# daviyan5/ninpol

Measured on AMD Instinct MI355X. Metric: Mnodes/s interpolated (GLS, 10M-cell hex mesh) + achieved HBM GB/s vs peak, higher is better.
Workload: dtype f64

## Files before the change

ninpol_amd/csrc/abi_apply.hip:

```cpp
#include <hipcub/hipcub.hpp>

#include "abi_internal.hpp"
#include "gls_adjoint.hpp"

using namespace nin;

int nin::ensure_transpose_index(DeviceGrid &d, hipStream_t stream) {
    if (d.tr_cell_ptr) return NIN_OK;
    const int32_t E = d.v.n_elems, nnz = (int32_t)d.nnz_e;
    int32_t *&ptr = d.tr_cell_ptr, *&pos = d.tr_cell_pos, *&node = d.tr_cell_node;
    DevTmp<int32_t> cells_sorted;
    DevTmp<void> tmp;
    size_t tmp_bytes = 0;
    int end_bit = 1;
    while (end_bit < 31 && (int64_t{1} << end_bit) < (int64_t)E) ++end_bit;
    int rc = dev_alloc(d, &ptr, (size_t)E + 1);
    if (!rc) rc = dev_alloc(d, &pos, (size_t)nnz);
    if (!rc) rc = dev_alloc(d, &node, (size_t)nnz);
    auto step = [&](hipError_t e) { if (e != hipSuccess && rc == NIN_OK) rc = fail(NIN_EHIP, "transpose index: %s", hipGetErrorString(e)); return rc == NIN_OK; };
    if (!rc && nnz > 0) {
        if (step(hipMalloc((void **)&cells_sorted, (size_t)nnz * sizeof(int32_t))) &&
            step(launch_iota(node, nnz, stream) ? hipErrorLaunchFailure : hipSuccess) &&
            step(hipcub::DeviceRadixSort::SortPairs(nullptr, tmp_bytes, d.v.esup, cells_sorted.p, node, pos, nnz, 0, end_bit, stream)) &&
            step(hipMalloc(&tmp, tmp_bytes)) &&
// ... 18 lines not shown
                     double *dev_neumann_ws, void *stream_) {
    if (!g || !dev_u_cells || !dev_node_values || !dev_neumann_ws) return fail(NIN_EINVAL, "NULL argument");
    if (n_fields < 1) return fail(NIN_EINVAL, "n_fields must be >= 1");
    DeviceGrid &d = g->d;
    if (int rc = on_device(g, kHintWeights)) return rc;
    HIP_TRY(hipSetDevice(d.device));
    hipStream_t stream = static_cast<hipStream_t>(stream_);
    if (int rc = ensure_apply_weights(d)) return rc;
    const DeviceGrid::GlsList &cube = d.plan[gk::hex8];
    if (method == NIN_METHOD_GLS && cube.count > 0 && d.noncube_nodes_ready && getenv("NIN_APPLY_NO_FUSION") == nullptr) {
        int rc = weights_ready(d, method);
        if (rc) return rc;
        HIP_TRY(hipMemsetAsync(d.gls_queue, 0, kGlsQueueInts * sizeof(int32_t), stream));
        rc = gls_side_begin(d, -1, 1, d.apply_weights, dev_neumann_ws, stream);
        if (!rc) rc = launch_gls_hex8mf_apply(d.v, cube.nodes, reinterpret_cast<const int32_t *>(cube.desc), cube.count, 1, dev_u_cells, n_fields,
                                              dev_node_values, dev_neumann_ws, d.gls_queue + gls_plan_row(gk::hex8).counter, stream);
        if (!rc) rc = gls_main(d, -1, false, gls_only(), 1, d.apply_weights, dev_neumann_ws, stream);
        if (!rc) rc = launch_apply_list(d.v, d.apply_weights, dev_u_cells, n_fields, dev_node_values, d.noncube_nodes, d.noncube_count, stream);
        if (rc) return fail(rc, "launch failed: %s", hipGetErrorString(hipGetLastError()));
        return NIN_OK;
    }
    int rc = nin_weights_device(g, method, nullptr, 0, 1, d.apply_weights, dev_neumann_ws, stream_);
    if (rc) return rc;
    rc = n_fields == 1 ? launch_apply(d.v, d.apply_weights, dev_u_cells, dev_node_values, (int32_t)g->h.mx_elems_per_point, d.nnz_e, stream)
                       : launch_apply_fields(d.v, d.apply_weights, dev_u_cells, n_fields, dev_node_values, (int32_t)g->h.mx_elems_per_point, d.nnz_e, stream);
    if (rc) return fail(rc, "launch failed");
    return NIN_OK;
}

int nin_apply_fields_host(nin_grid *g, int method, const double *u_cells, int32_t n_fields, double *node_values,
                          double *neumann_ws) {
// ... 336 lines not shown
```

ninpol_amd/csrc/abi_plan.hip:

```cpp
#include <hipcub/hipcub.hpp>
#include <cmath>

#include "abi_internal.hpp"
#include "hex8_desc.hpp"
#include "mfw_desc.hpp"
#include "mfg_desc.hpp"
#include "mfx_desc.hpp"
#include "quad4_desc.hpp"

using namespace nin;

namespace {

#ifndef NIN_LOCALITY_RUN
#define NIN_LOCALITY_RUN 16
#endif
constexpr int kLocalityRun = NIN_LOCALITY_RUN;
__device__ __forceinline__ uint32_t spread10(uint32_t v) {
    v = (v | (v << 16)) & 0x030000FFu;
    v = (v | (v << 8)) & 0x0300F00Fu;
    v = (v | (v << 4)) & 0x030C30C3u;
    v = (v | (v << 2)) & 0x09249249u;
    return v;
}
// ... 76 lines not shown
        default: return 0;
    }
}

int launch_plan_kernel(const DeviceGrid &d, GlsKernel k, const int32_t *nodes, const uint32_t *desc, int32_t count, int add_neumann,
                       double *out, double *nws, hipStream_t stream) {
    const GlsPlanRow r = gls_plan_row(k);
    const DeviceGrid::GlsList &l = d.plan[k];
    int32_t *queue = r.counter >= 0 ? d.gls_queue + r.counter : nullptr;
    const int32_t *idesc = reinterpret_cast<const int32_t *>(desc);
    switch (r.family) {
        case GlsFamily::block: return launch_gls_block(d.v, nodes, count, l.waves, l.col_slots, l.lds_bytes, add_neumann, out, nws, queue, stream);
        case GlsFamily::scratch:
            return launch_gls_class(d.v, nodes, count, 0, l.rows_per_lane, add_neumann, out, nws, d.gls_scratch, d.gls_scratch_stride,
                                    d.gls_scratch_slots, stream);
        case GlsFamily::hex8: return launch_gls_hex8mf(d.v, nodes, idesc, count, add_neumann, out, nws, queue, stream);
        case GlsFamily::mfw: return launch_gls_mfw(d.v, nodes, desc, count, r.sub, add_neumann, out, nws, queue, stream);
        case GlsFamily::small: return launch_gls_small(d.v, nodes, count, r.sub, add_neumann, out, nws, stream);
        case GlsFamily::quad4: return launch_gls_quad4(d.v, nodes, idesc, count, add_neumann, out, nws, stream);
        case GlsFamily::mfx: return launch_gls_mfx(d.v, nodes, desc, count, r.sub, add_neumann, out, nws, queue, stream);
        case GlsFamily::mfg: return launch_gls_mfg(d.v, nodes, desc, count, add_neumann, out, nws, queue, d.mfg_tiles, d.mfg_slots, stream);
    }
    return NIN_EINVAL;
}

}

int nin::build_gls_plan(nin_grid *g) {
    DeviceGrid &d = g->d;
    const int64_t P = g->h.n_points;
    int rc;
// ... 59 lines not shown
        const int32_t *lp = nullptr;
        if ((rc = dev_upload(d, &lp, lists[k]))) return rc;
        l.nodes = const_cast<int32_t *>(lp);
        if (k == gk::hex8 && locality && (rc = locality_order(d, l.nodes, l.count, d.chunk_node))) return rc;
        if (const int words = gls_plan_row(k).desc_words) {
            if ((rc = dev_alloc(d, &l.desc, (size_t)l.count * words))) return rc;
            if (launch_plan_desc(d, GlsKernel(k), l.nodes, l.count, l.desc, nullptr)) return fail(NIN_EHIP, "descriptor kernel of plan kernel %d", k);
        }
    }
    if (d.plan[gk::mfg_tiles].count) {
        d.mfg_slots = std::min<int32_t>(d.plan[gk::mfg_tiles].count, kMfgResidentWaves);
        if ((rc = dev_alloc(d, &d.mfg_tiles, (size_t)d.mfg_slots * kMfgSlotDoubles))) return rc;
    }
    d.gls_too_large = rows_max[gk::scratch] > 1024;
    if ((rc = dev_alloc(d, &d.gls_queue, (size_t)kGlsQueueInts))) return rc;
    if (d.plan[gk::scratch].count) {
        d.gls_scratch_slots = std::min<int32_t>(d.plan[gk::scratch].count, 512);
        d.gls_scratch_stride = need_max[gk::scratch] / 8;
        if ((rc = dev_alloc(d, &d.gls_scratch, (size_t)d.gls_scratch_slots * d.gls_scratch_stride))) return rc;
    }
    const char *mn = getenv("NIN_E2E_MIN_NODES");
    d.chunkable = P >= (mn ? atoll(mn) : 64 * 1024) && P >= 64 * K && getenv("NIN_E2E_NO_PIPELINE") == nullptr;
    for (int c = 0; c < kGlsClasses; ++c)
        if (d.plan[c].count == P) { d.plan[c].nodes = nullptr; d.chunkable = false; }
    return NIN_OK;
}

static constexpr GlsKernel kSideOrder[] = {gk::mfg_tiles, gk::scratch};
static constexpr GlsKernel kMainOrder[] = {gk::hex8,     gk::mfw_large, gk::mfw_small, gk::mfw_general, gk::small4,       gk::small8,
                                           gk::small12,  gk::quad4,     gk::mfx_6x10,  gk::mfx_7x11,    gk::mfx_8x13,     gk::mfx_9x15,
                                           gk::mfx_10x16, gk::mfx_boundary, gk::mfx_4x7, gk::mfx_7x12,  gk::mfg_tiles,    gk::block1,
                                           gk::block2,   gk::block4,    gk::block8,    gk::scratch};
static constexpr bool main_order_is_complete() {
    unsigned seen = 0;
    for (GlsKernel k : kMainOrder) seen |= 1u << k;
    return sizeof kMainOrder / sizeof kMainOrder[0] == kGlsPlanKernels && seen == (1u << kGlsPlanKernels) - 1;
}
static_assert(main_order_is_complete(), "kMainOrder must name every kernel of the plan once");
static bool on_side_stream(GlsKernel k) { return std::find(std::begin(kSideOrder), std::end(kSideOrder), k) != std::end(kSideOrder); }

struct PlanRange { const int32_t *nodes; const uint32_t *desc; int32_t count; };
static PlanRange plan_range(const DeviceGrid &d, GlsKernel k, int piece) {
    const auto &l = d.plan[k];
    const int32_t b = piece < 0 ? 0 : l.chunk_off[piece], n = (piece < 0 ? l.count : l.chunk_off[piece + 1]) - b;
    return {l.nodes ? l.nodes + b : nullptr, l.desc ? l.desc + (size_t)gls_plan_row(k).desc_words * b : nullptr, n};
// ... 67 lines not shown
                       double *dev_csr_data, double *dev_neumann_ws, void *stream_) {
    if (!g || !dev_csr_data || !dev_neumann_ws) return fail(NIN_EINVAL, "NULL argument");
    DeviceGrid &d = g->d;
    int rc = on_device(g, kHintWeights);
    if (!rc) rc = weights_ready(d, method);
    if (rc) return rc;
    hipStream_t stream = static_cast<hipStream_t>(stream_);
    HIP_TRY(hipSetDevice(d.device));
    const int64_t P = g->h.n_points;
    const bool all = targets == nullptr;
    if (!all && n_targets < 0) return fail(NIN_EINVAL, "negative n_targets");
    if (all) {
        if (method == NIN_METHOD_IDW) rc = launch_idw(d.v, nullptr, (int32_t)P, (int32_t)g->h.mx_elems_per_point, d.nnz_e, dev_csr_data, dev_neumann_ws, stream);
        else if (method == NIN_METHOD_LS) rc = launch_ls(d.v, nullptr, (int32_t)P, (int32_t)g->h.mx_elems_per_point, d.nnz_e, dev_csr_data, dev_neumann_ws, stream);
        else {
            HIP_TRY(hipMemsetAsync(d.gls_queue, 0, kGlsQueueInts * sizeof(int32_t), stream));
            const int only = gls_only();
            if (only < 0) rc = gls_side_begin(d, -1, add_neumann, dev_csr_data, dev_neumann_ws, stream);
            if (!rc) rc = gls_main(d, -1, true, only, add_neumann, dev_csr_data, dev_neumann_ws, stream);
        }
        if (rc) return fail(rc, "kernel launch failed: %s", hipGetErrorString(hipGetLastError()));
        return NIN_OK;
    }
    for (int64_t i = 0; i < n_targets; ++i)
        if (targets[i] < 0 || targets[i] >= P) return fail(NIN_EINVAL, "target %lld out of range", (long long)targets[i]);
    HIP_TRY(hipMemsetAsync(dev_csr_data, 0, (size_t)d.nnz_e * 8, stream));
    HIP_TRY(hipMemsetAsync(dev_neumann_ws, 0, (size_t)P * 8, stream));
    if (n_targets == 0) return NIN_OK;
    const bool gls = method == NIN_METHOD_GLS;
    std::vector<int32_t> lists[kGlsPlanKernels];
    for (int64_t i = 0; i < n_targets; ++i) lists[gls ? gls_class_kernel(g->node_class[targets[i]]) : 0].push_back((int32_t)targets[i]);
// ... 158 lines not shown
```

ninpol_amd/csrc/device_grid.hpp:

```cpp
#pragma once
#include <cstdint>
#include <string>
#include <vector>

#include "gls_plan.hpp"

namespace nin {

struct GridView {
    int32_t n_points, n_elems, n_faces, dim;
    const int32_t *esup_ptr;
    const int32_t *esup;
    const int32_t *fsup_ptr;
    const int32_t *fsup;
    const double *coords;
    const double *centroids;
    const double *centroids4;
    const int32_t *face_cells;
    const double *face_center;
    const float *face_normal;
    const double *perm;
    const double *diff_mag;
    const uint8_t *flags;
};
// ... 6 lines not shown
    return ((doubles * 8 + 15) / 16) * 16;
}
NIN_HD inline int gls_node_class(int64_t ne, int64_t nf, int64_t nbf, bool force_global, int64_t *bytes, int64_t *rows,
                                 int64_t *cols) {
    const int64_t m = ne + 3 * (nf - nbf) + nbf, n = 3 * ne + 1;
    int c = kGlsClasses - 1;
    int64_t b = ((((ne + 1) >> 1) + n + m * n) * 8 + 15) / 16 * 16;
    for (int k = 0; k < kGlsClasses - 1 && !force_global && n <= 256; ++k) {
        const int64_t need = gls_block_lds_bytes(ne, m, n, gls_class_waves(k));
        if (need <= gls_class_budget(k)) { c = k; b = need; break; }
    }
    *bytes = b; *rows = m; *cols = n;
    return c;
}

struct DeviceGrid {
    int device = -1;
    GridView v{};
    int64_t nnz_e = 0, nnz_f = 0;
    bool fields_set = false, have_perm = false;
    bool prebuilt = false;
    std::vector<void *> allocs;

    static constexpr int kE2eChunks = 4;
    int32_t chunk_node[kE2eChunks + 1] = {0, 0, 0, 0, 0};
    bool chunkable = false;
    struct GlsList {
        int32_t count = 0;
        int32_t *nodes = nullptr;
        uint32_t *desc = nullptr;
        int32_t chunk_off[kE2eChunks + 1] = {};
        int32_t lds_bytes = 0;
        int32_t waves = 1;
        int32_t col_slots = 1;
        int32_t rows_per_lane = 1;
    } plan[kGlsPlanKernels];
    double *mfg_tiles = nullptr;
    int32_t mfg_slots = 0;
    const int32_t *noncube_nodes = nullptr;
    int32_t noncube_count = 0;
    bool noncube_nodes_ready = false;
    double *gls_scratch = nullptr;
    int64_t gls_scratch_stride = 0;
    int32_t gls_scratch_slots = 0;
    int32_t *gls_queue = nullptr;
    double *e2e_weights = nullptr, *e2e_nws = nullptr, *e2e_data = nullptr;
    int32_t *e2e_cnt = nullptr, *e2e_ptr = nullptr, *e2e_indices = nullptr;
    void *e2e_tmp = nullptr;
    size_t e2e_tmp_bytes = 0;
    double *apply_weights = nullptr;
    int32_t *tr_cell_ptr = nullptr, *tr_cell_pos = nullptr, *tr_cell_node = nullptr;
    struct AdjBin {
        int32_t count = 0;
        int32_t *nodes = nullptr;
        int64_t bytes = 0;
    } adj_bin[4];
    bool adj_ready = false;
    double *adj_contrib = nullptr, *adj_scratch = nullptr;
    int64_t adj_scratch_stride = 0;
    int32_t adj_scratch_slots = 0;
// ... 36 lines not shown
```

ninpol_amd/csrc/gls_plan.hpp:

```cpp
#pragma once
#include <cstdint>

#ifdef __HIPCC__
#define NIN_HD __host__ __device__
#else
#define NIN_HD
#endif

namespace nin {

constexpr int kGlsClasses = 5;

constexpr int kGlsPlanKernels = 22;
namespace gk {
enum GlsKernel : int {
    block1, block2, block4, block8, scratch,
    hex8,
    mfw_large, mfw_small, mfw_general,
    small4, small8, small12,
    quad4,
    mfx_6x10, mfx_7x11, mfx_8x13, mfx_9x15, mfx_10x16,
    mfx_boundary,
    mfg_tiles,
    mfx_4x7,
// ... 7 lines not shown
    scratch,
    hex8,
    mfw,
    small,
    quad4,
    mfx,
    mfg,
};

constexpr int kGlsQueueLine = 16;
constexpr int kGlsQueueHex8 = 0, kGlsQueueHex8Lines = 8;
constexpr int kGlsQueueBlock = 1;
constexpr int kGlsQueueMfw = 5;
constexpr int kGlsQueueMfx = 8, kGlsQueueMfxLists = 8;
constexpr int kGlsQueueMfg = 8 * kGlsQueueLine;
constexpr int kGlsQueueInts = 9 * kGlsQueueLine;
static_assert(kGlsQueueBlock > kGlsQueueHex8 && kGlsQueueBlock + (kGlsClasses - 1) <= kGlsQueueMfw, "block counters overlap");
static_assert(kGlsQueueMfw + 3 <= kGlsQueueMfx, "mfw counters overlap the mfx counters");
static_assert(kGlsQueueMfx + kGlsQueueMfxLists <= kGlsQueueLine, "the block / mfw / mfx counters must stay between hex8's ints 0 and 16");
static_assert(kGlsQueueMfg % kGlsQueueLine == 0 && kGlsQueueMfg / kGlsQueueLine >= kGlsQueueHex8 / kGlsQueueLine + kGlsQueueHex8Lines,
              "the mfg counter must lie on none of hex8's eight lines");
static_assert(kGlsQueueMfg < kGlsQueueInts, "the mfg counter lies outside the block");

struct GlsPlanRow {
    GlsFamily family;
    int8_t sub;
    uint8_t class_byte;
    int16_t desc_words;
    int16_t fdq_word;
    int16_t counter;
};
// ... 87 lines not shown
```

ninpol_amd/csrc/kernels_gls_hex8mf.hip:

```cpp
#include <hip/hip_runtime.h>

#include <cstdio>
#include <cstdlib>

#include "device_grid.hpp"
#include "gls_device_math.hpp"
#include "hex8_desc.hpp"
#include "launch.hpp"

namespace nin {

namespace {

using namespace glsmath;

__device__ __forceinline__ double quad_sum(double v) {
    v += dpp_mov<0xB1>(v);
    v += dpp_mov<0x4E>(v);
    return v;
}
template <int L>
__device__ __forceinline__ double quad_bcast(double v) { return dpp_mov<L * 0x55>(v); }

constexpr int NPW = 16;
// ... 86 lines not shown
        const bool own = R0 >= 0 && r >= R0 && r < R0 + 3;
        const double v = own ? fma(w0, P[r][0], b[own ? r - R0 : 0]) : w0 * P[r][0];
        fill[r - 3] = fma(w2, P[r][2], fma(w1, P[r][1], v));
    }
}

__device__ __forceinline__ void w2_dma16(const void *gptr, uint32_t *row) {
    __builtin_amdgcn_global_load_lds((const __attribute__((address_space(1))) void *)gptr, (__attribute__((address_space(3))) void *)row, 16, 0, 0);
}
__device__ __forceinline__ void w2_dma_wait() {
    __builtin_amdgcn_sched_barrier(0);
    asm volatile("s_waitcnt vmcnt(0)" ::: "memory");
    __builtin_amdgcn_sched_barrier(0);
}
constexpr int W2_REC_ROW = 256;
__device__ __forceinline__ void w2_stage_rec(const int32_t *rec, int32_t wg, int32_t count, int nd, int l, uint32_t *rows_r) {
    const int32_t idx = wg * NPW + nd;
    const uint32_t sel = (uint32_t)((idx >= 0 && idx < count) ? idx : count - 1);
    const int32_t *r = rec + kHex8LaneWords * (4 * (size_t)sel + l);
    w2_dma16(r, rows_r);
    w2_dma16(r + 4, rows_r + W2_REC_ROW);
}
struct W2Geo {
    double Ke[9], dme, ce[3];
    double Ko[9], dmo, co[3];
    double fc[3][3];
    float fn[3][3];
    double xv[3];
    uint32_t flags;
};
__device__ __forceinline__ void w2_stage_d(const GridView &g, const uint32_t *rows_r, int lane, W2Geo &q) {
    const uint4 ra = *reinterpret_cast<const uint4 *>(rows_r + 4 * lane);
    const uint4 rb = *reinterpret_cast<const uint4 *>(rows_r + W2_REC_ROW + 4 * lane);
#pragma unroll
    for (int t = 0; t < 3; ++t) q.xv[t] = g.coords[3 * (size_t)ra.x + t];
    q.flags = g.flags[ra.x];
    const uint32_t ce = ra.z, co = ra.w;
#pragma unroll
    for (int k = 0; k < 9; ++k) { q.Ke[k] = g.perm[9 * (size_t)ce + k]; q.Ko[k] = g.perm[9 * (size_t)co + k]; }
    q.dme = g.diff_mag[ce];
    q.dmo = g.diff_mag[co];
#pragma unroll
    for (int t = 0; t < 3; ++t) { q.ce[t] = g.centroids[3 * (size_t)ce + t]; q.co[t] = g.centroids[3 * (size_t)co + t]; }
#pragma unroll
    for (int i = 0; i < 3; ++i) {
        const uint32_t f = i == 0 ? rb.x : i == 1 ? rb.y : rb.z;
#pragma unroll
        for (int t = 0; t < 3; ++t) { q.fn[i][t] = g.face_normal[3 * (size_t)f + t]; q.fc[i][t] = g.face_center[3 * (size_t)f + t]; }
    }
}
template <int I>
__device__ __forceinline__ double w2_across(double v) { return dpp_mov<I == 0 ? 0x40 : I == 1 ? 0xA5 : 0xFE>(v); }

#ifndef W2_D_STEP
#define W2_D_STEP 6
#endif
static_assert(W2_D_STEP >= 0 && W2_D_STEP <= 12, "the geometry is requested in phase 2");

#ifdef NIN_W2_TRACE
__device__ unsigned long long nin_w2_trace[4096 * 4];
#endif
template <bool APPLY>
__global__ __launch_bounds__(256, 2) void nin_gls_hex8w2_kernel(GridView g, const int32_t *__restrict__ nodes,
                                                                const int32_t *__restrict__ desc, int32_t count,
                                                                int add_neumann, double *__restrict__ out,
                                                                double *__restrict__ nws, int32_t *__restrict__ queue,
                                                                const double *__restrict__ u_cells, int32_t n_fields,
                                                                double *__restrict__ values) {
    __shared__ __attribute__((aligned(16))) double lds_all[4][W2_WAVE_DOUBLES];
    static_assert(W2_WAVE_DOUBLES % 2 == 0, "a wave's slots begin on a 16-byte boundary (the records' rows)");
    __shared__ double tau_tab[TAU_TAB_DOUBLES];
    static_assert(2 * (sizeof(double) * (4 * W2_WAVE_DOUBLES + TAU_TAB_DOUBLES)) <= 160 * 1024, "two workgroups per CU");
    tau_table_to_lds(tau_tab);
    __syncthreads();
    const lds_cdouble_ptr tau_lds = (lds_cdouble_ptr)tau_tab;
    const int lane = threadIdx.x & 63, wave = threadIdx.x >> 6;
    const int l = lane & 3, nd = lane >> 2;
    double *const L = lds_all[wave] + lane;
    double *const wbuf = lds_all[wave] + W2_SLOTS * 64;
    uint32_t *const rows_r = reinterpret_cast<uint32_t *>(lds_all[wave] + 13 * 64);

    const int32_t n_groups = (count + NPW - 1) / NPW;
    int32_t wg_lo, wg_end;
    int32_t *q;
    if ((gridDim.x & 7) == 0) {
        const int32_t xcd = blockIdx.x & 7, per = (n_groups + 7) / 8;
        wg_lo = xcd * per;
        wg_end = (xcd + 1) * per < n_groups ? (xcd + 1) * per : n_groups;
        q = queue + kGlsQueueLine * xcd;
    } else {
        wg_lo = 0;
        wg_end = n_groups;
        q = queue;
    }
    int32_t ticket = 0;
    if (lane == 0) ticket = atomicAdd(q, 1);
    int32_t wg = wg_lo + __builtin_amdgcn_readfirstlane(ticket);
    if (lane == 0) ticket = atomicAdd(q, 1);
    int32_t wg_next = wg_lo + __builtin_amdgcn_readfirstlane(ticket);
    W2Geo geo;
    w2_stage_rec(desc, wg, count, nd, l, rows_r);
    w2_dma_wait();
    w2_stage_d(g, rows_r, lane, geo);
#ifdef NIN_MF_STAMPS
#ifndef NIN_MF_STAMP_PASS
#define NIN_MF_STAMP_PASS 8
#endif
    unsigned long long stamps[8];
    int n_stamp = 0, pass_no = 0;
#define NIN_MF_STAMP() do { if (n_stamp < 8) { __builtin_amdgcn_sched_barrier(0); stamps[n_stamp++] = __builtin_amdgcn_s_memtime(); __builtin_amdgcn_s_waitcnt(0xC07F); __builtin_amdgcn_sched_barrier(0); } } while (0)
#else
#define NIN_MF_STAMP() do { } while (0)
#endif
#ifdef NIN_W2_TRACE
    const unsigned long long trace_t0 = __builtin_amdgcn_s_memrealtime();
    unsigned trace_passes = 0;
#endif
    while (wg < wg_end) {
#ifdef NIN_W2_TRACE
        ++trace_passes;
#endif
#ifdef NIN_MF_STAMPS
        n_stamp = 0;
#endif
        NIN_MF_STAMP();
        const bool valid = wg * NPW + nd < count;
        __builtin_amdgcn_s_waitcnt(0x0F70);
#ifdef NIN_MF_STAMP_SPLIT
        NIN_MF_STAMP();
#define NIN_MF_STAMP_BACK() do { } while (0)
// ... 6 lines not shown
        const bool is_neu = (geo.flags & 2) != 0;
        __builtin_amdgcn_sched_barrier(0);

        double P[10][3], de[3], dod[3], nb0[3][3], sav[3][2][3];
        {
            const double dme = geo.dme;
#pragma unroll
            for (int t = 0; t < 3; ++t) {
                de[t] = geo.ce[t] - xv[t];
                dod[t] = geo.co[t] - xv[t];
                P[0][t] = de[t];
            }
#pragma unroll
            for (int i = 0; i < 3; ++i) {
                const uint32_t w = dsc >> (6 + 8 * i);
                const double N0 = (double)geo.fn[i][0], N1 = (double)geo.fn[i][1], N2 = (double)geo.fn[i][2];
                const double T0 = xv[0] - geo.fc[i][0], T1 = xv[1] - geo.fc[i][1], T2 = xv[2] - geo.fc[i][2];
                const double U0 = N1 * T2 - N2 * T1, U1 = N2 * T0 - N0 * T2, U2 = N0 * T1 - N1 * T0;
                auto across = [&](double v) { return i == 0 ? w2_across<0>(v) : i == 1 ? w2_across<1>(v) : w2_across<2>(v); };
                const double dmn = across(geo.dmo);
                double eta = 0.0;
                eta = dme > eta ? dme : eta;
                eta = dmn > eta ? dmn : eta;
                const double tj = face_tau_tab_t<true>(U0 * U0 + U1 * U1 + U2 * U2, eta, tau_lds);
                const bool side_a = ((w >> 7) & 1) != 0;
                const double sg = side_a ? -1.0 : 1.0;
                double Kn[9];
#pragma unroll
                for (int k = 0; k < 9; ++k) Kn[k] = across(geo.Ko[k]);
#pragma unroll
                for (int t = 0; t < 3; ++t) {
                    P[1 + 3 * i][t] = sg * (geo.Ke[t * 3 + 0] * N0 + geo.Ke[t * 3 + 1] * N1 + geo.Ke[t * 3 + 2] * N2);
                    nb0[i][t] = -sg * (Kn[t * 3 + 0] * N0 + Kn[t * 3 + 1] * N1 + Kn[t * 3 + 2] * N2);
                }
                sav[i][0][0] = sg * T0; sav[i][0][1] = sg * T1; sav[i][0][2] = sg * T2;
                sav[i][1][0] = sg * (tj * U0); sav[i][1][1] = sg * (tj * U1); sav[i][1][2] = sg * (tj * U2);
#pragma unroll
                for (int t = 0; t < 3; ++t) { P[2 + 3 * i][t] = sav[i][0][t]; P[3 + 3 * i][t] = sav[i][1][t]; }
            }
        }
        NIN_MF_STAMP();
        if (lane == 0) ticket = atomicAdd(q, 1);
        __builtin_amdgcn_sched_barrier(0);
        double C[NR][NC];
        double u[9], se, F1[7][2], F2[7][3];
        {
            double g3[3], z[3];
            front_panel(P, de, g3, z);
            pin(z[0]); pin(z[1]); pin(z[2]);
            double cc[3];
            cc[0] = P[1][1] * P[1][0];
// ... 77 lines not shown
#pragma unroll
        for (int j = 0; j < 9; ++j) L[64 * j] = u[j];
        L[64 * 9] = se;
#pragma unroll
        for (int s = 0; s < 4; ++s) {
#pragma unroll
            for (int t = 0; t < 3; ++t) C[7][3 * s + t] = (l == s) ? dod[t] : 0.0;
        }
        C[7][12] = 1.0;
        __builtin_amdgcn_sched_barrier(0);

        double rinvq[3] = {0.0, 0.0, 0.0};
        NIN_MF_STAMP();
        __builtin_amdgcn_sched_barrier(0);
        __builtin_amdgcn_s_waitcnt(0xC07F);
        w2_stage_rec(desc, wg_next, count, nd, l, rows_r);
        __builtin_amdgcn_sched_barrier(0);
        P2LeanLoop<0, W2_D_STEP>::run(C, rinvq, l);
        NIN_MF_STAMP();
        __builtin_amdgcn_sched_barrier(0);
        w2_dma_wait();
        int32_t wg_after = wg_lo + __builtin_amdgcn_readfirstlane(ticket);
        asm volatile("" : "+s"(wg_after));
        __builtin_amdgcn_sched_barrier(0);
        w2_stage_d(g, rows_r, lane, geo);
        __builtin_amdgcn_sched_barrier(0);
        P2LeanLoop<W2_D_STEP, 12>::run(C, rinvq, l);
        NIN_MF_STAMP();
        double y[12], t3[3] = {C[0][12], C[1][12], C[2][12]};
        BackLoop<11>::run(C, rinvq, t3, y, l);
        NIN_MF_STAMP_BACK();
        double tail = 0.0;
#pragma unroll
        for (int r = 3; r < NR; ++r) tail = fma(C[r][12], C[r][12], tail);
        const double rr = quad_sum(tail);

        double re = 1.0 - L[64 * 9];
#pragma unroll
        for (int i = 0; i < 3; ++i) {
            const bool low = i < 3 - l;
// ... 6 lines not shown
        const double dsel = (l == 0) ? dots[0] : (l == 1) ? dots[1] : (l == 2) ? dots[2] : dots[3];
        const double ro = 1.0 - dsel;
        const double rri = fast_rcp(rr);
        double we = re * rri, wo = ro * rri;
        const bool ok = rr > 0.0;
        we = (ok && __builtin_isfinite(we)) ? we : 0.0;
        wo = (ok && __builtin_isfinite(wo)) ? wo : 0.0;

        wbuf[nd * 8 + (dsc & 7)] = we;
        wbuf[nd * 8 + ((dsc >> 3) & 7)] = wo;
        wave_lds_sync();
        const double nwv = is_neu ? wbuf[nd * 8 + 7] : 0.0;
        const double addv = add_neumann ? nwv : 0.0;
        const double o0 = wbuf[nd * 8 + 2 * l] + addv, o1 = wbuf[nd * 8 + 2 * l + 1] + addv;
        if (APPLY) {
            const size_t c0 = (size_t)g.esup[eb + 2 * l], c1 = (size_t)g.esup[eb + 2 * l + 1];
            for (int32_t f = 0; f < n_fields; ++f) {
                const double *uf = u_cells + (size_t)f * (size_t)g.n_elems;
                const double yv = quad_sum(fma(o1, uf[c1], o0 * uf[c0]));
                if (valid && l == 0) values[(size_t)f * (size_t)g.n_points + p] = yv;
            }
            if (valid && l == 0) nws[p] = nwv;
        } else if (valid) {
            out[eb + 2 * l] = o0;
            out[eb + 2 * l + 1] = o1;
            if (l == 0) nws[p] = nwv;
        }
        wave_lds_sync();
        NIN_MF_STAMP();
#ifdef NIN_MF_STAMPS
        if (blockIdx.x == 0 && threadIdx.x == 0 && ++pass_no == NIN_MF_STAMP_PASS)
            for (int i = 0; i < 8; ++i) nws[nodes[i]] = (double)(stamps[i] - stamps[0]);
#endif
        wg = wg_next;
        wg_next = wg_after;
    }
    w2_dma_wait();
#ifdef NIN_W2_TRACE
    if (lane == 0 && blockIdx.x < 1024) {
        unsigned long long *t = nin_w2_trace + 4 * ((size_t)blockIdx.x * 4 + wave);
        t[0] = trace_t0;
        t[1] = __builtin_amdgcn_s_memrealtime();
        t[2] = __builtin_amdgcn_s_getreg((4 << 0) | (0 << 6) | (31 << 11));
        t[3] = trace_passes;
    }
#endif
}

__global__ void k_hex8_desc(GridView g, const int32_t *__restrict__ nodes, int32_t count, int32_t *__restrict__ desc) {
    const int64_t i = (int64_t)blockIdx.x * blockDim.x + threadIdx.x;
    if (i >= count) return;
    int32_t d[kHex8DescWords] = {};
    (void)hex8_descriptor<true>(g, nodes ? nodes[i] : (int32_t)i, d);
    int4 *rec = reinterpret_cast<int4 *>(desc) + (kHex8DescWords / 4) * i;
#pragma unroll
    for (int w = 0; w < kHex8DescWords / 4; ++w) rec[w] = make_int4(d[4 * w], d[4 * w + 1], d[4 * w + 2], d[4 * w + 3]);
}

}

int launch_hex8_desc(const GridView &g, const int32_t *nodes, int32_t count, int32_t *desc, hipStream_t stream) {
    if (count <= 0) return 0;
    hipLaunchKernelGGL(k_hex8_desc, dim3((unsigned)((count + 255) / 256)), dim3(256), 0, stream, g, nodes, count, desc);
    return hipGetLastError() == hipSuccess ? 0 : -3;
}

int launch_gls_hex8mf(const GridView &g, const int32_t *nodes, const int32_t *desc, int32_t count, int add_neumann,
                      double *out, double *nws, int32_t *queue, hipStream_t stream) {
    if (count <= 0) return 0;
    int64_t blocks = ((int64_t)count + 4 * NPW - 1) / (4 * NPW);
    const char *cap_env = getenv("NIN_W2_BLOCKS");
    const int64_t cap2 = cap_env ? atoll(cap_env) : 512;
    if (blocks > cap2) blocks = cap2;
    if (blocks > 8) blocks &= ~(int64_t)7;
    if (getenv("NIN_DEBUG_OCCUPANCY") != nullptr) {
        int nb = -1;
        (void)hipOccupancyMaxActiveBlocksPerMultiprocessor(&nb, nin_gls_hex8w2_kernel<false>, 256, 0);
        fprintf(stderr, "nin_gls_hex8w2_kernel: %d workgroups per CU, %lld launched\n", nb, (long long)blocks);
    }
    hipLaunchKernelGGL(nin_gls_hex8w2_kernel<false>, dim3((unsigned)blocks), dim3(256), 0, stream, g, nodes, desc, count, add_neumann, out, nws, queue,
                       nullptr, 0, nullptr);
#ifdef NIN_W2_TRACE
    if (getenv("NIN_W2_TRACE_FILE") != nullptr) {
        static int calls = 0;
        if (++calls == 6) {
            (void)hipStreamSynchronize(stream);
            static unsigned long long host[4096 * 4];
            (void)hipMemcpyFromSymbol(host, HIP_SYMBOL(nin_w2_trace), sizeof(host));
            FILE *f = fopen(getenv("NIN_W2_TRACE_FILE"), "w");
            for (int64_t b = 0; b < blocks * 4 && b < 4096; ++b)
                fprintf(f, "%lld %llu %llu %llx %llu\n", (long long)b, host[4 * b], host[4 * b + 1], host[4 * b + 2], host[4 * b + 3]);
            fclose(f);
        }
    }
#endif
    return hipGetLastError() == hipSuccess ? 0 : -3;
}

int launch_gls_hex8mf_apply(const GridView &g, const int32_t *nodes, const int32_t *desc, int32_t count, int add_neumann,
                            const double *u_cells, int32_t n_fields, double *values, double *nws, int32_t *queue, hipStream_t stream) {
    if (count <= 0) return 0;
    int64_t blocks = ((int64_t)count + 4 * NPW - 1) / (4 * NPW);
    if (blocks > 512) blocks = 512;
    if (blocks > 8) blocks &= ~(int64_t)7;
    hipLaunchKernelGGL(nin_gls_hex8w2_kernel<true>, dim3((unsigned)blocks), dim3(256), 0, stream, g, nodes, desc, count, add_neumann,
                       nullptr, nws, queue, u_cells, n_fields, values);
    return hipGetLastError() == hipSuccess ? 0 : -3;
}

const char *kernel_name_gls_hex8mf() { return "nin_gls_hex8w2_kernel<false>"; }

}
```

ninpol_amd/csrc/launch.hpp:

```cpp
#pragma once
#include <hip/hip_runtime.h>

#include <cstdint>

#include "device_grid.hpp"

namespace nin {

#ifdef __HIPCC__
template <auto KERN>
inline int allow_dynamic_lds(size_t bytes) {
    if (bytes <= 48 * 1024) return 0;
    static size_t allowed[64] = {};
    int dev = 0;
    (void)hipGetDevice(&dev);
    size_t &a = allowed[dev & 63];
    if (bytes > a) {
        if (hipFuncSetAttribute(reinterpret_cast<const void *>(KERN), hipFuncAttributeMaxDynamicSharedMemorySize, (int)bytes) != hipSuccess) return -3;
        a = bytes;
    }
    return 0;
}
#endif

int launch_idw(const GridView &g, const int32_t *targets, int32_t n_targets, int32_t mx_row, int64_t nnz, double *out, double *nws,
               hipStream_t stream);
int launch_ls(const GridView &g, const int32_t *targets, int32_t n_targets, int32_t mx_row, int64_t nnz, double *out, double *nws,
              hipStream_t stream);
int launch_gls_class(const GridView &g, const int32_t *nodes, int32_t count, int32_t lds_bytes,
                     int32_t rows_per_lane, int add_neumann, double *out, double *nws,
                     double *scratch, int64_t scratch_stride, int32_t scratch_slots, hipStream_t stream);
int launch_gls_block(const GridView &g, const int32_t *nodes, int32_t count, int32_t waves, int32_t col_slots,
                     int32_t lds_bytes, int add_neumann, double *out, double *nws, int32_t *queue, hipStream_t stream);
const char *kernel_name_gls_block();
int launch_hex8_desc(const GridView &g, const int32_t *nodes, int32_t count, int32_t *desc, hipStream_t stream);
int launch_gls_hex8mf(const GridView &g, const int32_t *nodes, const int32_t *desc, int32_t count, int add_neumann,
                      double *out, double *nws, int32_t *queue, hipStream_t stream);
int launch_gls_hex8mf_apply(const GridView &g, const int32_t *nodes, const int32_t *desc, int32_t count, int add_neumann,
                            const double *u_cells, int32_t n_fields, double *values, double *nws, int32_t *queue, hipStream_t stream);
const char *kernel_name_gls_hex8mf();
int launch_mfw_desc(const GridView &g, const int32_t *nodes, int32_t count, uint32_t *desc, hipStream_t stream);
int launch_gls_mfw(const GridView &g, const int32_t *nodes, const uint32_t *desc, int32_t count, int kind, int add_neumann,
                   double *out, double *nws, int32_t *queue, hipStream_t stream);
const char *kernel_name_gls_mfw();
int launch_mfx_desc(const GridView &g, const int32_t *nodes, int32_t count, uint32_t *desc, hipStream_t stream);
int launch_gls_mfx(const GridView &g, const int32_t *nodes, const uint32_t *desc, int32_t count, int cls, int add_neumann, double *out,
                   double *nws, int32_t *queue, hipStream_t stream);
const char *kernel_name_gls_mfx();
int launch_mfg_desc(const GridView &g, const int32_t *nodes, int32_t count, uint32_t *desc, hipStream_t stream);
int launch_gls_mfg(const GridView &g, const int32_t *nodes, const uint32_t *desc, int32_t count, int add_neumann, double *out, double *nws,
                   int32_t *queue, double *tiles, int32_t n_slots, hipStream_t stream);
const char *kernel_name_gls_mfg();
int launch_quad4_desc(const GridView &g, const int32_t *nodes, int32_t count, int32_t *desc, hipStream_t stream);
int launch_gls_quad4(const GridView &g, const int32_t *nodes, const int32_t *desc, int32_t count, int add_neumann, double *out,
// ... 107 lines not shown
```

Measured before the change: 2268.

## Use 32-bit byte offsets in hex8 kernel and self-reset work counters

The hex8 GLS kernel gains a template path that computes gather addresses with 32-bit byte offsets, using shift-add helpers, whenever the mesh sizes fit in 4 GiB. This is meant to reduce 64-bit address arithmetic and VGPR pressure. The kernel also counts finished waves and resets its own queue counters, so the per-call memset can be skipped when hex8 is the only queued kernel. Separately, the face sign is folded into the normal once instead of being applied to each product, and the main launch order now runs the small kernels before hex8. The added atomic reset logic and reordering bring correctness and scheduling risk.

Result: no change. 2283, median of 6 (+0.7%).

```diff
diff --git a/ninpol_amd/csrc/abi_apply.hip b/ninpol_amd/csrc/abi_apply.hip
--- a/ninpol_amd/csrc/abi_apply.hip
+++ b/ninpol_amd/csrc/abi_apply.hip
@@ -56,7 +56,7 @@
         HIP_TRY(hipMemsetAsync(d.gls_queue, 0, kGlsQueueInts * sizeof(int32_t), stream));
         rc = gls_side_begin(d, -1, 1, d.apply_weights, dev_neumann_ws, stream);
         if (!rc) rc = launch_gls_hex8mf_apply(d.v, cube.nodes, reinterpret_cast<const int32_t *>(cube.desc), cube.count, 1, dev_u_cells, n_fields,
-                                              dev_node_values, dev_neumann_ws, d.gls_queue + gls_plan_row(gk::hex8).counter, stream);
+                                              dev_node_values, dev_neumann_ws, d.gls_queue + gls_plan_row(gk::hex8).counter, d.w2_off32, stream);
         if (!rc) rc = gls_main(d, -1, false, gls_only(), 1, d.apply_weights, dev_neumann_ws, stream);
         if (!rc) rc = launch_apply_list(d.v, d.apply_weights, dev_u_cells, n_fields, dev_node_values, d.noncube_nodes, d.noncube_count, stream);
         if (rc) return fail(rc, "launch failed: %s", hipGetErrorString(hipGetLastError()));
diff --git a/ninpol_amd/csrc/abi_plan.hip b/ninpol_amd/csrc/abi_plan.hip
--- a/ninpol_amd/csrc/abi_plan.hip
+++ b/ninpol_amd/csrc/abi_plan.hip
@@ -114,7 +114,7 @@
         case GlsFamily::scratch:
             return launch_gls_class(d.v, nodes, count, 0, l.rows_per_lane, add_neumann, out, nws, d.gls_scratch, d.gls_scratch_stride,
                                     d.gls_scratch_slots, stream);
-        case GlsFamily::hex8: return launch_gls_hex8mf(d.v, nodes, idesc, count, add_neumann, out, nws, queue, stream);
+        case GlsFamily::hex8: return launch_gls_hex8mf(d.v, nodes, idesc, count, add_neumann, out, nws, queue, d.w2_off32, stream);
         case GlsFamily::mfw: return launch_gls_mfw(d.v, nodes, desc, count, r.sub, add_neumann, out, nws, queue, stream);
         case GlsFamily::small: return launch_gls_small(d.v, nodes, count, r.sub, add_neumann, out, nws, stream);
         case GlsFamily::quad4: return launch_gls_quad4(d.v, nodes, idesc, count, add_neumann, out, nws, stream);
@@ -204,6 +204,11 @@
     }
     d.gls_too_large = rows_max[gk::scratch] > 1024;
     if ((rc = dev_alloc(d, &d.gls_queue, (size_t)kGlsQueueInts))) return rc;
+    if (hipMemset(d.gls_queue, 0, kGlsQueueInts * sizeof(int32_t)) != hipSuccess) return fail(NIN_EHIP, "hipMemset of the work counters");
+    d.queue_hex8_only = true;
+    for (int k = 0; k < kGlsPlanKernels; ++k)
+        if (k != gk::hex8 && gls_plan_row(k).counter >= 0 && d.plan[k].count > 0) d.queue_hex8_only = false;
+    d.w2_off32 = w2_off32_ok(d.v, d.nnz_e);
     if (d.plan[gk::scratch].count) {
         d.gls_scratch_slots = std::min<int32_t>(d.plan[gk::scratch].count, 512);
         d.gls_scratch_stride = need_max[gk::scratch] / 8;
@@ -217,8 +222,8 @@
 }
 
 static constexpr GlsKernel kSideOrder[] = {gk::mfg_tiles, gk::scratch};
-static constexpr GlsKernel kMainOrder[] = {gk::hex8,     gk::mfw_large, gk::mfw_small, gk::mfw_general, gk::small4,       gk::small8,
-                                           gk::small12,  gk::quad4,     gk::mfx_6x10,  gk::mfx_7x11,    gk::mfx_8x13,     gk::mfx_9x15,
+static constexpr GlsKernel kMainOrder[] = {gk::small4,   gk::small8,    gk::small12,   gk::quad4,       gk::hex8,         gk::mfw_large,
+                                           gk::mfw_small, gk::mfw_general, gk::mfx_6x10, gk::mfx_7x11,  gk::mfx_8x13,     gk::mfx_9x15,
                                            gk::mfx_10x16, gk::mfx_boundary, gk::mfx_4x7, gk::mfx_7x12,  gk::mfg_tiles,    gk::block1,
                                            gk::block2,   gk::block4,    gk::block8,    gk::scratch};
 static constexpr bool main_order_is_complete() {
@@ -316,7 +321,7 @@
         if (method == NIN_METHOD_IDW) rc = launch_idw(d.v, nullptr, (int32_t)P, (int32_t)g->h.mx_elems_per_point, d.nnz_e, dev_csr_data, dev_neumann_ws, stream);
         else if (method == NIN_METHOD_LS) rc = launch_ls(d.v, nullptr, (int32_t)P, (int32_t)g->h.mx_elems_per_point, d.nnz_e, dev_csr_data, dev_neumann_ws, stream);
         else {
-            HIP_TRY(hipMemsetAsync(d.gls_queue, 0, kGlsQueueInts * sizeof(int32_t), stream));
+            if (!d.queue_hex8_only) HIP_TRY(hipMemsetAsync(d.gls_queue, 0, kGlsQueueInts * sizeof(int32_t), stream));
             const int only = gls_only();
             if (only < 0) rc = gls_side_begin(d, -1, add_neumann, dev_csr_data, dev_neumann_ws, stream);
             if (!rc) rc = gls_main(d, -1, true, only, add_neumann, dev_csr_data, dev_neumann_ws, stream);
diff --git a/ninpol_amd/csrc/device_grid.hpp b/ninpol_amd/csrc/device_grid.hpp
--- a/ninpol_amd/csrc/device_grid.hpp
+++ b/ninpol_amd/csrc/device_grid.hpp
@@ -44,6 +44,12 @@
     return c;
 }
 
+constexpr uint64_t kW2Off32Bytes = 1ull << 32;
+inline bool w2_off32_ok(const GridView &v, int64_t nnz_e) {
+    const uint64_t P = (uint64_t)v.n_points, E = (uint64_t)v.n_elems, F = (uint64_t)v.n_faces;
+    return P * 128 < kW2Off32Bytes && E * 72 < kW2Off32Bytes && F * 24 < kW2Off32Bytes && (uint64_t)nnz_e * 4 < kW2Off32Bytes;
+}
+
 struct DeviceGrid {
     int device = -1;
     GridView v{};
@@ -74,6 +80,8 @@
     int64_t gls_scratch_stride = 0;
     int32_t gls_scratch_slots = 0;
     int32_t *gls_queue = nullptr;
+    bool w2_off32 = false;
+    bool queue_hex8_only = false;
     double *e2e_weights = nullptr, *e2e_nws = nullptr, *e2e_data = nullptr;
     int32_t *e2e_cnt = nullptr, *e2e_ptr = nullptr, *e2e_indices = nullptr;
     void *e2e_tmp = nullptr;
diff --git a/ninpol_amd/csrc/gls_plan.hpp b/ninpol_amd/csrc/gls_plan.hpp
--- a/ninpol_amd/csrc/gls_plan.hpp
+++ b/ninpol_amd/csrc/gls_plan.hpp
@@ -45,7 +45,9 @@
 constexpr int kGlsQueueMfw = 5;
 constexpr int kGlsQueueMfx = 8, kGlsQueueMfxLists = 8;
 constexpr int kGlsQueueMfg = 8 * kGlsQueueLine;
+constexpr int kGlsQueueHex8Done = kGlsQueueMfg + 1;
 constexpr int kGlsQueueInts = 9 * kGlsQueueLine;
+static_assert(kGlsQueueHex8Done > kGlsQueueMfg && kGlsQueueHex8Done + kGlsQueueHex8Lines <= kGlsQueueInts, "hex8's count of finished waves lies outside the block");
 static_assert(kGlsQueueBlock > kGlsQueueHex8 && kGlsQueueBlock + (kGlsClasses - 1) <= kGlsQueueMfw, "block counters overlap");
 static_assert(kGlsQueueMfw + 3 <= kGlsQueueMfx, "mfw counters overlap the mfx counters");
 static_assert(kGlsQueueMfx + kGlsQueueMfxLists <= kGlsQueueLine, "the block / mfw / mfx counters must stay between hex8's ints 0 and 16");
diff --git a/ninpol_amd/csrc/kernels_gls_hex8mf.hip b/ninpol_amd/csrc/kernels_gls_hex8mf.hip
--- a/ninpol_amd/csrc/kernels_gls_hex8mf.hip
+++ b/ninpol_amd/csrc/kernels_gls_hex8mf.hip
@@ -124,10 +124,12 @@
     __builtin_amdgcn_sched_barrier(0);
 }
 constexpr int W2_REC_ROW = 256;
+template <bool OFF32>
 __device__ __forceinline__ void w2_stage_rec(const int32_t *rec, int32_t wg, int32_t count, int nd, int l, uint32_t *rows_r) {
     const int32_t idx = wg * NPW + nd;
     const uint32_t sel = (uint32_t)((idx >= 0 && idx < count) ? idx : count - 1);
-    const int32_t *r = rec + kHex8LaneWords * (4 * (size_t)sel + l);
+    const int32_t *r = OFF32 ? reinterpret_cast<const int32_t *>(reinterpret_cast<const char *>(rec) + ((4 * sel + (uint32_t)l) * (4u * kHex8LaneWords)))
+                             : rec + kHex8LaneWords * (4 * (size_t)sel + l);
     w2_dma16(r, rows_r);
     w2_dma16(r + 4, rows_r + W2_REC_ROW);
 }
@@ -139,9 +141,40 @@
     double xv[3];
     uint32_t flags;
 };
+template <class T>
+__device__ __forceinline__ const T *w2_at(const T *base, uint32_t byte_off) {
+    return reinterpret_cast<const T *>(reinterpret_cast<const char *>(base) + byte_off);
+}
+__device__ __forceinline__ uint32_t w2_x3(uint32_t x) { asm volatile("" : "+v"(x)); uint32_t r = (x << 1) + x; asm volatile("" : "+v"(r)); return r; }
+__device__ __forceinline__ uint32_t w2_x9(uint32_t x) { asm volatile("" : "+v"(x)); uint32_t r = (x << 3) + x; asm volatile("" : "+v"(r)); return r; }
+template <bool OFF32>
 __device__ __forceinline__ void w2_stage_d(const GridView &g, const uint32_t *rows_r, int lane, W2Geo &q) {
     const uint4 ra = *reinterpret_cast<const uint4 *>(rows_r + 4 * lane);
     const uint4 rb = *reinterpret_cast<const uint4 *>(rows_r + W2_REC_ROW + 4 * lane);
+    if (OFF32) {
+        const double *xp = w2_at(g.coords, w2_x3(ra.x << 3));
+#pragma unroll
+        for (int t = 0; t < 3; ++t) q.xv[t] = xp[t];
+        q.flags = *w2_at(g.flags, ra.x);
+        const uint32_t ce8 = ra.z << 3, co8 = ra.w << 3;
+        const double *ke = w2_at(g.perm, w2_x9(ce8)), *ko = w2_at(g.perm, w2_x9(co8));
+#pragma unroll
+        for (int k = 0; k < 9; ++k) { q.Ke[k] = ke[k]; q.Ko[k] = ko[k]; }
+        q.dme = *w2_at(g.diff_mag, ce8);
+        q.dmo = *w2_at(g.diff_mag, co8);
+        const double *xe = w2_at(g.centroids, w2_x3(ce8)), *xo = w2_at(g.centroids, w2_x3(co8));
+#pragma unroll
+        for (int t = 0; t < 3; ++t) { q.ce[t] = xe[t]; q.co[t] = xo[t]; }
+#pragma unroll
+        for (int i = 0; i < 3; ++i) {
+            const uint32_t f12 = w2_x3((i == 0 ? rb.x : i == 1 ? rb.y : rb.z) << 2);
+            const float *fn = w2_at(g.face_normal, f12);
+            const double *fc = w2_at(g.face_center, f12 << 1);
+#pragma unroll
+            for (int t = 0; t < 3; ++t) { q.fn[i][t] = fn[t]; q.fc[i][t] = fc[t]; }
+        }
+        return;
+    }
 #pragma unroll
     for (int t = 0; t < 3; ++t) q.xv[t] = g.coords[3 * (size_t)ra.x + t];
     q.flags = g.flags[ra.x];
@@ -168,9 +201,9 @@
 static_assert(W2_D_STEP >= 0 && W2_D_STEP <= 12, "the geometry is requested in phase 2");
 
 #ifdef NIN_W2_TRACE
-__device__ unsigned long long nin_w2_trace[4096 * 4];
-#endif
-template <bool APPLY>
+__device__ unsigned long long nin_w2_trace[4096 * 6];
+#endif
+template <bool APPLY, bool OFF32>
 __global__ __launch_bounds__(256, 2) void nin_gls_hex8w2_kernel(GridView g, const int32_t *__restrict__ nodes,
                                                                 const int32_t *__restrict__ desc, int32_t count,
                                                                 int add_neumann, double *__restrict__ out,
@@ -192,16 +225,21 @@
 
     const int32_t n_groups = (count + NPW - 1) / NPW;
     int32_t wg_lo, wg_end;
-    int32_t *q;
+    int32_t *q, *q_done;
+    int32_t q_waves;
     if ((gridDim.x & 7) == 0) {
         const int32_t xcd = blockIdx.x & 7, per = (n_groups + 7) / 8;
         wg_lo = xcd * per;
         wg_end = (xcd + 1) * per < n_groups ? (xcd + 1) * per : n_groups;
         q = queue + kGlsQueueLine * xcd;
+        q_done = queue + (kGlsQueueHex8Done - kGlsQueueHex8) + xcd;
+        q_waves = (int32_t)(gridDim.x >> 3) * 4;
     } else {
         wg_lo = 0;
         wg_end = n_groups;
         q = queue;
+        q_done = queue + (kGlsQueueHex8Done - kGlsQueueHex8);
+        q_waves = (int32_t)gridDim.x * 4;
     }
     int32_t ticket = 0;
     if (lane == 0) ticket = atomicAdd(q, 1);
@@ -209,9 +247,9 @@
     if (lane == 0) ticket = atomicAdd(q, 1);
     int32_t wg_next = wg_lo + __builtin_amdgcn_readfirstlane(ticket);
     W2Geo geo;
-    w2_stage_rec(desc, wg, count, nd, l, rows_r);
+    w2_stage_rec<OFF32>(desc, wg, count, nd, l, rows_r);
     w2_dma_wait();
-    w2_stage_d(g, rows_r, lane, geo);
+    w2_stage_d<OFF32>(g, rows_r, lane, geo);
 #ifdef NIN_MF_STAMPS
 #ifndef NIN_MF_STAMP_PASS
 #define NIN_MF_STAMP_PASS 8
@@ -223,7 +261,7 @@
 #define NIN_MF_STAMP() do { } while (0)
 #endif
 #ifdef NIN_W2_TRACE
-    const unsigned long long trace_t0 = __builtin_amdgcn_s_memrealtime();
+    const unsigned long long trace_t0 = __builtin_amdgcn_s_memrealtime(), trace_c0 = __builtin_amdgcn_s_memtime();
     unsigned trace_passes = 0;
 #endif
     while (wg < wg_end) {
@@ -260,7 +298,9 @@
 #pragma unroll
             for (int i = 0; i < 3; ++i) {
                 const uint32_t w = dsc >> (6 + 8 * i);
-                const double N0 = (double)geo.fn[i][0], N1 = (double)geo.fn[i][1], N2 = (double)geo.fn[i][2];
+                const bool side_a = ((w >> 7) & 1) != 0;
+                const double sg = side_a ? -1.0 : 1.0;
+                const double N0 = sg * (double)geo.fn[i][0], N1 = sg * (double)geo.fn[i][1], N2 = sg * (double)geo.fn[i][2];
                 const double T0 = xv[0] - geo.fc[i][0], T1 = xv[1] - geo.fc[i][1], T2 = xv[2] - geo.fc[i][2];
                 const double U0 = N1 * T2 - N2 * T1, U1 = N2 * T0 - N0 * T2, U2 = N0 * T1 - N1 * T0;
                 auto across = [&](double v) { return i == 0 ? w2_across<0>(v) : i == 1 ? w2_across<1>(v) : w2_across<2>(v); };
@@ -269,18 +309,16 @@
                 eta = dme > eta ? dme : eta;
                 eta = dmn > eta ? dmn : eta;
                 const double tj = face_tau_tab_t<true>(U0 * U0 + U1 * U1 + U2 * U2, eta, tau_lds);
-                const bool side_a = ((w >> 7) & 1) != 0;
-                const double sg = side_a ? -1.0 : 1.0;
                 double Kn[9];
 #pragma unroll
                 for (int k = 0; k < 9; ++k) Kn[k] = across(geo.Ko[k]);
 #pragma unroll
                 for (int t = 0; t < 3; ++t) {
-                    P[1 + 3 * i][t] = sg * (geo.Ke[t * 3 + 0] * N0 + geo.Ke[t * 3 + 1] * N1 + geo.Ke[t * 3 + 2] * N2);
-                    nb0[i][t] = -sg * (Kn[t * 3 + 0] * N0 + Kn[t * 3 + 1] * N1 + Kn[t * 3 + 2] * N2);
+                    P[1 + 3 * i][t] = geo.Ke[t * 3 + 0] * N0 + geo.Ke[t * 3 + 1] * N1 + geo.Ke[t * 3 + 2] * N2;
+                    nb0[i][t] = -(Kn[t * 3 + 0] * N0 + Kn[t * 3 + 1] * N1 + Kn[t * 3 + 2] * N2);
                 }
                 sav[i][0][0] = sg * T0; sav[i][0][1] = sg * T1; sav[i][0][2] = sg * T2;
-                sav[i][1][0] = sg * (tj * U0); sav[i][1][1] = sg * (tj * U1); sav[i][1][2] = sg * (tj * U2);
+                sav[i][1][0] = tj * U0; sav[i][1][1] = tj * U1; sav[i][1][2] = tj * U2;
 #pragma unroll
                 for (int t = 0; t < 3; ++t) { P[2 + 3 * i][t] = sav[i][0][t]; P[3 + 3 * i][t] = sav[i][1][t]; }
             }
@@ -388,7 +426,7 @@
         NIN_MF_STAMP();
         __builtin_amdgcn_sched_barrier(0);
         __builtin_amdgcn_s_waitcnt(0xC07F);
-        w2_stage_rec(desc, wg_next, count, nd, l, rows_r);
+        w2_stage_rec<OFF32>(desc, wg_next, count, nd, l, rows_r);
         __builtin_amdgcn_sched_barrier(0);
         P2LeanLoop<0, W2_D_STEP>::run(C, rinvq, l);
         NIN_MF_STAMP();
@@ -397,7 +435,7 @@
         int32_t wg_after = wg_lo + __builtin_amdgcn_readfirstlane(ticket);
         asm volatile("" : "+s"(wg_after));
         __builtin_amdgcn_sched_barrier(0);
-        w2_stage_d(g, rows_r, lane, geo);
+        w2_stage_d<OFF32>(g, rows_r, lane, geo);
         __builtin_amdgcn_sched_barrier(0);
         P2LeanLoop<W2_D_STEP, 12>::run(C, rinvq, l);
         NIN_MF_STAMP();
@@ -434,10 +472,12 @@
         const double addv = add_neumann ? nwv : 0.0;
         const double o0 = wbuf[nd * 8 + 2 * l] + addv, o1 = wbuf[nd * 8 + 2 * l + 1] + addv;
         if (APPLY) {
-            const size_t c0 = (size_t)g.esup[eb + 2 * l], c1 = (size_t)g.esup[eb + 2 * l + 1];
+            const int32_t *er = OFF32 ? w2_at(g.esup, (eb + 2 * l) << 2) : g.esup + (eb + 2 * l);
+            const uint32_t c0 = (uint32_t)er[0], c1 = (uint32_t)er[1];
             for (int32_t f = 0; f < n_fields; ++f) {
                 const double *uf = u_cells + (size_t)f * (size_t)g.n_elems;
-                const double yv = quad_sum(fma(o1, uf[c1], o0 * uf[c0]));
+                const double u0 = OFF32 ? *w2_at(uf, c0 << 3) : uf[(size_t)c0], u1 = OFF32 ? *w2_at(uf, c1 << 3) : uf[(size_t)c1];
+                const double yv = quad_sum(fma(o1, u1, o0 * u0));
                 if (valid && l == 0) values[(size_t)f * (size_t)g.n_points + p] = yv;
             }
             if (valid && l == 0) nws[p] = nwv;
@@ -456,11 +496,17 @@
         wg_next = wg_after;
     }
     w2_dma_wait();
+    if (lane == 0 && atomicAdd(q_done, 1) == q_waves - 1) {
+        atomicExch(q, 0);
+        atomicExch(q_done, 0);
+    }
 #ifdef NIN_W2_TRACE
     if (lane == 0 && blockIdx.x < 1024) {
-        unsigned long long *t = nin_w2_trace + 4 * ((size_t)blockIdx.x * 4 + wave);
+        unsigned long long *t = nin_w2_trace + 6 * ((size_t)blockIdx.x * 4 + wave);
         t[0] = trace_t0;
         t[1] = __builtin_amdgcn_s_memrealtime();
+        t[4] = trace_c0;
+        t[5] = __builtin_amdgcn_s_memtime();
         t[2] = __builtin_amdgcn_s_getreg((4 << 0) | (0 << 6) | (31 << 11));
         t[3] = trace_passes;
     }
@@ -485,9 +531,15 @@
     return hipGetLastError() == hipSuccess ? 0 : -3;
 }
 
+static bool w2_use_off32(bool off32, int32_t count) {
+    const char *e = getenv("NIN_W2_WIDE_OFFSETS");
+    return off32 && (uint64_t)count * (4 * kHex8DescWords) < kW2Off32Bytes && !(e && *e && *e != '0');
+}
+
 int launch_gls_hex8mf(const GridView &g, const int32_t *nodes, const int32_t *desc, int32_t count, int add_neumann,
-                      double *out, double *nws, int32_t *queue, hipStream_t stream) {
+                      double *out, double *nws, int32_t *queue, bool off32, hipStream_t stream) {
     if (count <= 0) return 0;
+    off32 = w2_use_off32(off32, count);
     int64_t blocks = ((int64_t)count + 4 * NPW - 1) / (4 * NPW);
     const char *cap_env = getenv("NIN_W2_BLOCKS");
     const int64_t cap2 = cap_env ? atoll(cap_env) : 512;
@@ -495,21 +547,27 @@
     if (blocks > 8) blocks &= ~(int64_t)7;
     if (getenv("NIN_DEBUG_OCCUPANCY") != nullptr) {
         int nb = -1;
-        (void)hipOccupancyMaxActiveBlocksPerMultiprocessor(&nb, nin_gls_hex8w2_kernel<false>, 256, 0);
-        fprintf(stderr, "nin_gls_hex8w2_kernel: %d workgroups per CU, %lld launched\n", nb, (long long)blocks);
-    }
-    hipLaunchKernelGGL(nin_gls_hex8w2_kernel<false>, dim3((unsigned)blocks), dim3(256), 0, stream, g, nodes, desc, count, add_neumann, out, nws, queue,
-                       nullptr, 0, nullptr);
+        if (off32) (void)hipOccupancyMaxActiveBlocksPerMultiprocessor(&nb, nin_gls_hex8w2_kernel<false, true>, 256, 0);
+        else (void)hipOccupancyMaxActiveBlocksPerMultiprocessor(&nb, nin_gls_hex8w2_kernel<false, false>, 256, 0);
+        fprintf(stderr, "nin_gls_hex8w2_kernel (%d-bit offsets): %d workgroups per CU, %lld launched\n", off32 ? 32 : 64, nb, (long long)blocks);
+    }
+    if (off32)
+        hipLaunchKernelGGL((nin_gls_hex8w2_kernel<false, true>), dim3((unsigned)blocks), dim3(256), 0, stream, g, nodes, desc, count, add_neumann, out,
+                           nws, queue, nullptr, 0, nullptr);
+    else
+        hipLaunchKernelGGL((nin_gls_hex8w2_kernel<false, false>), dim3((unsigned)blocks), dim3(256), 0, stream, g, nodes, desc, count, add_neumann, out,
+                           nws, queue, nullptr, 0, nullptr);
 #ifdef NIN_W2_TRACE
     if (getenv("NIN_W2_TRACE_FILE") != nullptr) {
         static int calls = 0;
         if (++calls == 6) {
             (void)hipStreamSynchronize(stream);
-            static unsigned long long host[4096 * 4];
+            static unsigned long long host[4096 * 6];
             (void)hipMemcpyFromSymbol(host, HIP_SYMBOL(nin_w2_trace), sizeof(host));
             FILE *f = fopen(getenv("NIN_W2_TRACE_FILE"), "w");
             for (int64_t b = 0; b < blocks * 4 && b < 4096; ++b)
-                fprintf(f, "%lld %llu %llu %llx %llu\n", (long long)b, host[4 * b], host[4 * b + 1], host[4 * b + 2], host[4 * b + 3]);
+                fprintf(f, "%lld %llu %llu %llx %llu %llu %llu\n", (long long)b, host[6 * b], host[6 * b + 1], host[6 * b + 2], host[6 * b + 3],
+                        host[6 * b + 4], host[6 * b + 5]);
             fclose(f);
         }
     }
@@ -518,16 +576,22 @@
 }
 
 int launch_gls_hex8mf_apply(const GridView &g, const int32_t *nodes, const int32_t *desc, int32_t count, int add_neumann,
-                            const double *u_cells, int32_t n_fields, double *values, double *nws, int32_t *queue, hipStream_t stream) {
+                            const double *u_cells, int32_t n_fields, double *values, double *nws, int32_t *queue, bool off32,
+                            hipStream_t stream) {
     if (count <= 0) return 0;
+    off32 = w2_use_off32(off32, count) && (uint64_t)n_fields * (uint64_t)g.n_elems * 8 < kW2Off32Bytes;
     int64_t blocks = ((int64_t)count + 4 * NPW - 1) / (4 * NPW);
     if (blocks > 512) blocks = 512;
     if (blocks > 8) blocks &= ~(int64_t)7;
-    hipLaunchKernelGGL(nin_gls_hex8w2_kernel<true>, dim3((unsigned)blocks), dim3(256), 0, stream, g, nodes, desc, count, add_neumann,
-                       nullptr, nws, queue, u_cells, n_fields, values);
+    if (off32)
+        hipLaunchKernelGGL((nin_gls_hex8w2_kernel<true, true>), dim3((unsigned)blocks), dim3(256), 0, stream, g, nodes, desc, count, add_neumann,
+                           nullptr, nws, queue, u_cells, n_fields, values);
+    else
+        hipLaunchKernelGGL((nin_gls_hex8w2_kernel<true, false>), dim3((unsigned)blocks), dim3(256), 0, stream, g, nodes, desc, count, add_neumann,
+                           nullptr, nws, queue, u_cells, n_fields, values);
     return hipGetLastError() == hipSuccess ? 0 : -3;
 }
 
-const char *kernel_name_gls_hex8mf() { return "nin_gls_hex8w2_kernel<false>"; }
-
-}
+const char *kernel_name_gls_hex8mf() { return "nin_gls_hex8w2_kernel<false, true>"; }
+
+}
diff --git a/ninpol_amd/csrc/launch.hpp b/ninpol_amd/csrc/launch.hpp
--- a/ninpol_amd/csrc/launch.hpp
+++ b/ninpol_amd/csrc/launch.hpp
@@ -35,9 +35,10 @@
 const char *kernel_name_gls_block();
 int launch_hex8_desc(const GridView &g, const int32_t *nodes, int32_t count, int32_t *desc, hipStream_t stream);
 int launch_gls_hex8mf(const GridView &g, const int32_t *nodes, const int32_t *desc, int32_t count, int add_neumann,
-                      double *out, double *nws, int32_t *queue, hipStream_t stream);
+                      double *out, double *nws, int32_t *queue, bool off32, hipStream_t stream);
 int launch_gls_hex8mf_apply(const GridView &g, const int32_t *nodes, const int32_t *desc, int32_t count, int add_neumann,
-                            const double *u_cells, int32_t n_fields, double *values, double *nws, int32_t *queue, hipStream_t stream);
+                            const double *u_cells, int32_t n_fields, double *values, double *nws, int32_t *queue, bool off32,
+                            hipStream_t stream);
 const char *kernel_name_gls_hex8mf();
 int launch_mfw_desc(const GridView &g, const int32_t *nodes, int32_t count, uint32_t *desc, hipStream_t stream);
 int launch_gls_mfw(const GridView &g, const int32_t *nodes, const uint32_t *desc, int32_t count, int kind, int add_neumann,
```
